# 0xPabloxx/3d-pointcloud-orientation-estimation

Measured on AMD Instinct MI355X. Metric: clouds/sec fwd+bwd, pointnet_pp_vonMises N=1024, higher is better.
Workload: dtype f32; 1 GPU; configs[1]: models/pointnet_pp_vonMises.py single-peak KL, N=1024, batch=32 per GPU, fwd+loss+bwd+allreduce+Adam, random-init weights (seed 42), device-side centre sampling; per_gpu_batch=32, global_batch=32, points=1024, parallelism=single, launch=hipGraph(fwd+loss+bwd) + eager all-reduce/Adam (the update clears the gradients)

## Files before the change

### 3d-pointcloud-orientation-estimation_amd/csrc/gemm_wsd3_kernels.hip

```cpp
#include <stdlib.h>

#include "kernels.h"
#include "split_prims.h"

namespace pnpp {

typedef __attribute__((address_space(3))) volatile unsigned wd3_flag;
__device__ int g_wsd3_timeouts;
__device__ __forceinline__ bool wd3_wait(wd3_flag *f, unsigned target) {
    bool ok = true;
    unsigned spins = 0;
    while ((unsigned)__builtin_amdgcn_readfirstlane((int)*f) < target) {
        __builtin_amdgcn_s_sleep(1);
        if (++spins > (1u << 16)) {
            ok = false;
            break;
        }
    }
    asm volatile("" ::: "memory");
    return ok;
}
__device__ __forceinline__ void wd3_post(wd3_flag *f, unsigned v) {
    asm volatile("s_waitcnt lgkmcnt(0)" ::: "memory");
    *f = v;
}

#ifdef PNPP_STAMPS
__device__ unsigned long long g_wsd3_stamps[2][2][8];
#define WD3_STAMP(i)                                                   \
    if (st_on) {                                                       \
        const unsigned long long st_t = __builtin_amdgcn_s_memtime();  \
        st_acc[i] += st_t - st_last;                                   \
        st_last = st_t;                                                \
    }
#else
#define WD3_STAMP(i)
#endif

template <int KD, int BN, bool HANDOFF>
struct Wsd3Lds {
    static constexpr int WPLANE = BN * KD * 2, APLANE = 32 * 128, ABUF = 3 * APLANE, APAIR = 2 * ABUF, BFR = 2 * 3 * 64 * 16;
    static constexpr int OFF_IMG = 3 * WPLANE, OFF_CST = OFF_IMG + 4 * APAIR, OFF_BFR = OFF_CST + 3 * KD * 4;
    static constexpr int OFF_FLG = OFF_BFR + (HANDOFF ? 4 * BFR : 0), END = OFF_FLG + 64;
};

template <int KD, int BN, int AM>
__global__ void __launch_bounds__(512, 1)
gemm_wsd3_kernel(const AOperand A, const float *__restrict__ W, int ldw, int M, int Nout, int ncol, const Epilogue E) {
    constexpr int NC = KD / 64, CT = KD / 32;
    static_assert(BN == 32, "one column tile per workgroup: the consumer wave holds dW (KD x 32) and the dA tile");
    constexpr bool SPLITDW = true;
    constexpr int CTC = SPLITDW ? CT / 2 : CT;
    constexpr bool HANDOFF = KD == 128;
    constexpr bool DW2 = KD == 128 && AM == A_DZ_POOL;
    constexpr bool ACC2 = true;
    constexpr int WPITCH = KD * 2, WPLANE = BN * WPITCH;
    constexpr int APLANE = 32 * 128, ABUF = 3 * APLANE;
    constexpr int APAIR = 2 * ABUF;
    using LY = Wsd3Lds<KD, BN, HANDOFF>;
    constexpr int BFR = LY::BFR;
    constexpr int OFF_IMG = LY::OFF_IMG, OFF_CST = LY::OFF_CST, OFF_BFR = LY::OFF_BFR, OFF_FLG = LY::OFF_FLG;
    static_assert(NC % 2 == 0, "chunk k of a strip uses buffer k & 1");
    extern __shared__ __attribute__((aligned(16))) unsigned char lds3[];
    unsigned char *Wp = lds3;
    float *Tc = reinterpret_cast<float *>(lds3 + OFF_CST);
    const int tid = threadIdx.x, lane = tid & 63, wave = __builtin_amdgcn_readfirstlane(tid >> 6);
    const bool producer = wave < 4;
    const int pair = wave & 3;
    unsigned char *Ap = lds3 + OFF_IMG + pair * APAIR;
    uint4 *Bf = reinterpret_cast<uint4 *>(lds3 + OFF_BFR + pair * BFR) + lane;
    wd3_flag *f_ready = (wd3_flag *)(lds3 + OFF_FLG) + 2 * pair, *f_done = f_ready + 1;
    const int l31 = lane & 31, lh = lane >> 5;
    auto xw = [](int n) { return n & 15; };

    const int nworkers = gridDim.x / ncol;
    int col_blk = blockIdx.x % ncol, worker = blockIdx.x / ncol;
    if ((nworkers & 7) == 0) {
        const int xcd = blockIdx.x & 7, i = blockIdx.x >> 3;
        col_blk = i % ncol, worker = (i / ncol) * 8 + xcd;
    }
    const int n0 = col_blk * BN;
    const int nstrips = M / 32, stride = nworkers * 4;
    int strip = worker * 4 + pair;
    const __amdgpu_buffer_rsrc_t resNull = sp_buf_rsrc_null(A.z);
    const __amdgpu_buffer_rsrc_t resP = sp_buf_rsrc(E.zp);
    const unsigned oq = 4u * ((unsigned)(4 * lh) * (unsigned)Nout + (unsigned)(n0 + l31));
    auto quni = [&](int r) -> unsigned { return 4u * (unsigned)(((r & 3) + 8 * (r >> 2)) * Nout); };
    const float e_sc = E.scale[n0 + l31], e_sh = E.shift[n0 + l31];
    unsigned tbase[2];
    {
        const int gi = lane & 15, qq = gi >> 2, pp = gi & 3, g1 = (lane >> 4) & 1;
#pragma unroll
        for (int b = 0; b < 2; ++b) {
            const int r = 8 * b + 4 * lh + qq, ch = 2 * g1 + (pp >> 1);
            tbase[b] = (unsigned)(r * 128 + 16 * (ch ^ sp_swz_row(r)) + 8 * (pp & 1));
        }
    }
    auto tofs = [&](int it, int s, int b) -> unsigned { return (tbase[b] ^ (unsigned)(it * 64)) + (unsigned)(s * 2048); };
    auto act_fragments = [&](const float (&z)[16], uint4 (&bfr)[2][3]) {
        float act[16];
#pragma unroll
        for (int r = 0; r < 16; ++r) act[r] = fmaxf(fmaf(z[r], e_sc, e_sh), 0.f);
#pragma unroll
        for (int s = 0; s < 2; ++s) {
            f32x4 v0, v1;
            v0[0] = act[8 * s + 0], v0[1] = act[8 * s + 1], v0[2] = act[8 * s + 2], v0[3] = act[8 * s + 3];
            v1[0] = act[8 * s + 4], v1[1] = act[8 * s + 5], v1[2] = act[8 * s + 6], v1[3] = act[8 * s + 7];
            uint2 h0, m0, l0, h1, m1, l1;
            sp_split4(v0, h0, m0, l0);
            sp_split4(v1, h1, m1, l1);
            bfr[s][0] = make_uint4(h0.x, h0.y, h1.x, h1.y);
            bfr[s][1] = make_uint4(m0.x, m0.y, m1.x, m1.y);
            bfr[s][2] = make_uint4(l0.x, l0.y, l1.x, l1.y);
        }
    };
    auto dw_tile = [&](const unsigned char *Ab, int it, const uint4 (&bfr)[2][3], f32x16 &dwl, f32x16 &dwsm, auto last) {
#pragma unroll
        for (int s = 0; s < 2; ++s) {
            uint4 ta[3];
#pragma unroll
            for (int p = 0; p < 3; ++p) {
                const uint2 lo = sp_tr_b64(Ab + p * APLANE + tofs(it, s, 0)), hi = sp_tr_b64(Ab + p * APLANE + tofs(it, s, 1));
                ta[p] = make_uint4(lo.x, lo.y, hi.x, hi.y);
            }
            if (s == 1) last();
            const bf16x8 ah = sp_op(ta[0]), am = sp_op(ta[1]), al = sp_op(ta[2]);
            const bf16x8 bh = sp_op(bfr[s][0]), bm = sp_op(bfr[s][1]), bl = sp_op(bfr[s][2]);
            f32x16 d = DW2 ? dwsm : dwl;
            d = __builtin_amdgcn_mfma_f32_32x32x16_bf16(al, bh, d, 0, 0, 0);
            d = __builtin_amdgcn_mfma_f32_32x32x16_bf16(ah, bl, d, 0, 0, 0);
            d = __builtin_amdgcn_mfma_f32_32x32x16_bf16(am, bm, d, 0, 0, 0);
            d = __builtin_amdgcn_mfma_f32_32x32x16_bf16(am, bh, d, 0, 0, 0);
            d = __builtin_amdgcn_mfma_f32_32x32x16_bf16(ah, bm, d, 0, 0, 0);
            if constexpr (DW2) {
                dwsm = d;
                dwl = __builtin_amdgcn_mfma_f32_32x32x16_bf16(ah, bh, dwl, 0, 0, 0);
            } else {
                dwl = __builtin_amdgcn_mfma_f32_32x32x16_bf16(ah, bh, d, 0, 0, 0);
            }
        }
    };

    if (tid < 8) ((wd3_flag *)(lds3 + OFF_FLG))[tid] = 0u;
    for (int c = tid; c < KD; c += 512) {
        const float g = A.cst[c], mu = A.cst[A.C + c], is = A.cst[2 * A.C + c], c1 = A.cst[3 * A.C + c], c2 = A.cst[4 * A.C + c];
        const float a = -g * is * c2;
        Tc[c] = g, Tc[KD + c] = a, Tc[2 * KD + c] = -g * c1 - a * mu;
    }
    {
        constexpr int NWF = (KD / 4) * BN / 512;
        f32x4 tw[NWF];
#pragma unroll
        for (int j = 0; j < NWF; ++j) {
            const int f = tid + 512 * j, nl = f % BN, k4 = 4 * (f / BN);
#pragma unroll
            for (int e = 0; e < 4; ++e) tw[j][e] = W[(size_t)(k4 + e) * ldw + n0 + nl];
        }
#pragma unroll
        for (int j = 0; j < NWF; ++j) {
            const int f = tid + 512 * j, nl = f % BN, k4 = 4 * (f / BN);
            uint2 h, m, l;
            sp_split4(tw[j], h, m, l);
            unsigned char *dst = Wp + nl * WPITCH + 16 * ((k4 >> 3) ^ xw(nl)) + 2 * (k4 & 7);
            *reinterpret_cast<uint2 *>(dst) = h;
            *reinterpret_cast<uint2 *>(dst + WPLANE) = m;
            *reinterpret_cast<uint2 *>(dst + 2 * WPLANE) = l;
        }
    }
    __syncthreads();

#ifdef PNPP_STAMPS
    const bool st_on = blockIdx.x == 8 && pair == 0;
    unsigned long long st_acc[8] = {0, 0, 0, 0, 0, 0, 0, 0};
    unsigned long long st_last = __builtin_amdgcn_s_memtime();
#endif
    f32x16 dw[CTC], dws[DW2 ? CTC : 1];
    double s1 = 0.0, s2 = 0.0;
    bool timed_out = false;

    if (producer) {
        const int q = lane & 15, q4 = 4 * q, rb = lane >> 4;
        const __amdgpu_buffer_rsrc_t resZ = sp_buf_rsrc(A.z), resY = sp_buf_rsrc(A.a), resI = sp_buf_rsrc(A.arg);
        const unsigned oa0 = 4u * ((unsigned)rb * (unsigned)KD + (unsigned)q4);
        f32x4 rz[2][8], ry[AM == A_DZ ? 2 : 1][8], rdm[2];
        int4 rarg[2];
        auto fetch_chunk = [&](bool have, int s, int c) {
            const __amdgpu_buffer_rsrc_t rZ = have ? resZ : resNull, rY = have ? resY : resNull, rI = have ? resI : resNull;
            const unsigned so = (unsigned)s * (32u * KD * 4u) + 256u * (unsigned)c;
#pragma unroll
            for (int i = 0; i < 8; ++i) {
                rz[c & 1][i] = sp_buf_load4(rZ, oa0, so + (unsigned)i * (4u * KD * 4u));
                if constexpr (AM == A_DZ) ry[c & 1][i] = sp_buf_load4(rY, oa0, so + (unsigned)i * (4u * KD * 4u));
            }
            if constexpr (AM == A_DZ_POOL) {
                const unsigned sg = (unsigned)s * (KD * 4u) + 256u * (unsigned)c;
                rdm[c & 1] = sp_buf_load4(rY, 4u * (unsigned)q4, sg);
                rarg[c & 1] = __builtin_bit_cast(int4, sp_buf_load4(rI, 4u * (unsigned)q4, sg));
            }
        };
        float zn[16];
        {
            const bool have = strip < nstrips;
            fetch_chunk(have, strip, 0);
            fetch_chunk(have, strip, 1);
            const __amdgpu_buffer_rsrc_t rP = have ? resP : resNull;
#pragma unroll
            for (int r = 0; r < 16; ++r) zn[r] = sp_buf_load1(rP, oq, (unsigned)strip * (32u * (unsigned)Nout * 4u) + quni(r));
        }
        unsigned wofs[4];
#pragma unroll
        for (int i = 0; i < 4; ++i) wofs[i] = (unsigned)(rb * 128 + 16 * ((q >> 1) ^ sp_swz_row(rb + 4 * i)) + 8 * (q & 1));
        if constexpr (SPLITDW) {
#pragma unroll
            for (int i = 0; i < CTC; ++i)
#pragma unroll
                for (int r = 0; r < 16; ++r) dw[i][r] = 0.f;
            if constexpr (DW2) {
#pragma unroll
                for (int i = 0; i < CTC; ++i)
#pragma unroll
                    for (int r = 0; r < 16; ++r) dws[i][r] = 0.f;
            }
        }
        unsigned kbase = 0;
        for (; strip < nstrips; strip += stride, kbase += NC) {
            const bool more = strip + stride < nstrips;
            const int snext = strip + stride;
            uint4 bfr[2][3];
            act_fragments(zn, bfr);
            {
                const __amdgpu_buffer_rsrc_t nP = more ? resP : resNull;
                const unsigned sn_off = (unsigned)snext * (32u * (unsigned)Nout * 4u);
#pragma unroll
                for (int r = 0; r < 16; ++r) zn[r] = sp_buf_load1(nP, oq, sn_off + quni(r));
            }
            if constexpr (HANDOFF) {
                if (kbase >= 2) timed_out = timed_out || !wd3_wait(f_done, kbase - 1);
#pragma unroll
                for (int s = 0; s < 2; ++s)
#pragma unroll
                    for (int p3 = 0; p3 < 3; ++p3) Bf[(s * 3 + p3) * 64] = bfr[s][p3];
            }
#pragma unroll
            for (int c = 0; c < NC; ++c) {
                unsigned char *Ab = Ap + (c & 1) * ABUF;
                const float4 cg = *reinterpret_cast<const float4 *>(Tc + 64 * c + q4), ca = *reinterpret_cast<const float4 *>(Tc + KD + 64 * c + q4);
                const float4 cb = *reinterpret_cast<const float4 *>(Tc + 2 * KD + 64 * c + q4);
                f32x4 dm = {0.f, 0.f, 0.f, 0.f};
                int4 ar = make_int4(-1, -1, -1, -1);
                if constexpr (AM == A_DZ_POOL) dm = rdm[c & 1], ar = rarg[c & 1];
                float4 bt;
                bt.x = fmaf(cg.x, dm[0], cb.x), bt.y = fmaf(cg.y, dm[1], cb.y), bt.z = fmaf(cg.z, dm[2], cb.z), bt.w = fmaf(cg.w, dm[3], cb.w);
                auto dz4 = [&](int i) -> f32x4 {
                    const f32x4 z = rz[c & 1][i];
                    const int r = rb + 4 * i;
                    f32x4 v;
                    if constexpr (AM == A_DZ) {
                        const f32x4 dy = ry[c & 1][i];
                        v[0] = fmaf(cg.x, dy[0], fmaf(ca.x, z[0], cb.x)), v[1] = fmaf(cg.y, dy[1], fmaf(ca.y, z[1], cb.y));
                        v[2] = fmaf(cg.z, dy[2], fmaf(ca.z, z[2], cb.z)), v[3] = fmaf(cg.w, dy[3], fmaf(ca.w, z[3], cb.w));
                    } else {
                        v[0] = fmaf(ca.x, z[0], r == ar.x ? bt.x : cb.x), v[1] = fmaf(ca.y, z[1], r == ar.y ? bt.y : cb.y);
                        v[2] = fmaf(ca.z, z[2], r == ar.z ? bt.z : cb.z), v[3] = fmaf(ca.w, z[3], r == ar.w ? bt.w : cb.w);
                    }
                    return v;
                };
                if constexpr (AM == A_DZ_POOL && !SPLITDW) {
                    uint2 ph[8], pm[8], pl[8];
#pragma unroll
                    for (int i = 0; i < 8; ++i) sp_split4(dz4(i), ph[i], pm[i], pl[i]);
                    WD3_STAMP(0)
                    if (c + 2 < NC) fetch_chunk(true, strip, c + 2);
                    else fetch_chunk(more, snext, c + 2 - NC);
                    if (kbase + c >= 2) timed_out = timed_out || !wd3_wait(f_done, kbase + c - 1);
                    WD3_STAMP(1)
#pragma unroll
                    for (int i = 0; i < 8; ++i) {
                        unsigned char *dst = Ab + wofs[i & 3] + i * 512;
                        *reinterpret_cast<uint2 *>(dst) = ph[i];
                        *reinterpret_cast<uint2 *>(dst + APLANE) = pm[i];
                        *reinterpret_cast<uint2 *>(dst + 2 * APLANE) = pl[i];
                    }
                } else {
                    if (kbase + c >= 2) timed_out = timed_out || !wd3_wait(f_done, kbase + c - 1);
                    WD3_STAMP(1)
#pragma unroll
                    for (int i = 0; i < 8; ++i) {
                        uint2 h, m, l;
                        sp_split4(dz4(i), h, m, l);
                        unsigned char *dst = Ab + wofs[i & 3] + i * 512;
                        *reinterpret_cast<uint2 *>(dst) = h;
                        *reinterpret_cast<uint2 *>(dst + APLANE) = m;
                        *reinterpret_cast<uint2 *>(dst + 2 * APLANE) = l;
                    }
                    WD3_STAMP(0)
                    if (c + 2 < NC) fetch_chunk(true, strip, c + 2);
                    else fetch_chunk(more, snext, c + 2 - NC);
                }
                wd3_post(f_ready, kbase + c + 1);
                WD3_STAMP(2)
                if constexpr (SPLITDW) {
                    if (c >= NC / 2) {
#pragma unroll
                        for (int it = 0; it < 2; ++it) dw_tile(Ab, it, bfr, dw[2 * c + it - CTC], dws[DW2 ? 2 * c + it - CTC : 0], [] {});
                    }
                }
            }
        }
    } else {
#pragma unroll
        for (int i = 0; i < CTC; ++i)
#pragma unroll
            for (int r = 0; r < 16; ++r) dw[i][r] = 0.f;
        if constexpr (DW2) {
#pragma unroll
            for (int i = 0; i < CTC; ++i)
#pragma unroll
                for (int r = 0; r < 16; ++r) dws[i][r] = 0.f;
        }
        const __amdgpu_buffer_rsrc_t resC = sp_buf_rsrc(E.c);
        const float e_mu = E.mu[n0 + l31], e_is = E.istd[n0 + l31];
        float zq[16];
        const unsigned arow = (unsigned)(l31 * 128);
        const int ax = sp_swz_row(l31);
        const unsigned char *brow = Wp + l31 * WPITCH;
        const int bx = xw(l31);
        float zn[16];
        if constexpr (!HANDOFF) {
            const __amdgpu_buffer_rsrc_t rP = strip < nstrips ? resP : resNull;
#pragma unroll
            for (int r = 0; r < 16; ++r) zn[r] = sp_buf_load1(rP, oq, (unsigned)strip * (32u * (unsigned)Nout * 4u) + quni(r));
        }
        unsigned kbase = 0;
        for (; strip < nstrips; strip += stride, kbase += NC) {
            const bool more = strip + stride < nstrips;
            uint4 bfr[2][3];
            if constexpr (HANDOFF) {
                const unsigned sq_off = (unsigned)strip * (32u * (unsigned)Nout * 4u);
#pragma unroll
                for (int r = 0; r < 16; ++r) zq[r] = sp_buf_load1(resP, oq, sq_off + quni(r));
            } else {
#pragma unroll
                for (int r = 0; r < 16; ++r) zq[r] = zn[r];
                const __amdgpu_buffer_rsrc_t nP = more ? resP : resNull;
                const unsigned sn_off = (unsigned)(strip + stride) * (32u * (unsigned)Nout * 4u);
#pragma unroll
                for (int r = 0; r < 16; ++r) zn[r] = sp_buf_load1(nP, oq, sn_off + quni(r));
                act_fragments(zq, bfr);
            }
            f32x16 acc, accs;
#pragma unroll
            for (int r = 0; r < 16; ++r) acc[r] = 0.f;
            if constexpr (ACC2) {
#pragma unroll
                for (int r = 0; r < 16; ++r) accs[r] = 0.f;
            }
            WD3_STAMP(3)
#pragma unroll
            for (int c = 0; c < NC; ++c) {
                const unsigned char *Ab = Ap + (c & 1) * ABUF;
                timed_out = timed_out || !wd3_wait(f_ready, kbase + c + 1);
                if constexpr (HANDOFF) {
                    if (c == 0) {
#pragma unroll
                        for (int s = 0; s < 2; ++s)
#pragma unroll
                            for (int p3 = 0; p3 < 3; ++p3) bfr[s][p3] = Bf[(s * 3 + p3) * 64];
                    }
                }
                WD3_STAMP(4)
#pragma unroll
                for (int t = 0; t < 4; ++t) {
                    const int g = 2 * t + lh;
                    uint4 fa[3], fb[3];
#pragma unroll
                    for (int p = 0; p < 3; ++p) {
                        fa[p] = *reinterpret_cast<const uint4 *>(Ab + p * APLANE + arow + 16 * (g ^ ax));
                        fb[p] = *reinterpret_cast<const uint4 *>(brow + p * WPLANE + 16 * ((8 * c + g) ^ bx));
                    }
                    const bf16x8 ah = sp_op(fa[0]), am = sp_op(fa[1]), al = sp_op(fa[2]);
                    const bf16x8 bh = sp_op(fb[0]), bm = sp_op(fb[1]), bl = sp_op(fb[2]);
                    f32x16 d = ACC2 ? accs : acc;
                    d = __builtin_amdgcn_mfma_f32_32x32x16_bf16(al, bh, d, 0, 0, 0);
                    d = __builtin_amdgcn_mfma_f32_32x32x16_bf16(ah, bl, d, 0, 0, 0);
                    d = __builtin_amdgcn_mfma_f32_32x32x16_bf16(am, bm, d, 0, 0, 0);
                    d = __builtin_amdgcn_mfma_f32_32x32x16_bf16(am, bh, d, 0, 0, 0);
                    d = __builtin_amdgcn_mfma_f32_32x32x16_bf16(ah, bm, d, 0, 0, 0);
                    if constexpr (ACC2) {
                        accs = d;
                        acc = __builtin_amdgcn_mfma_f32_32x32x16_bf16(ah, bh, acc, 0, 0, 0);
                    } else {
                        acc = __builtin_amdgcn_mfma_f32_32x32x16_bf16(ah, bh, d, 0, 0, 0);
                    }
                }
                WD3_STAMP(5)
                if (!SPLITDW || c < NC / 2) {
                    dw_tile(Ab, 0, bfr, dw[2 * c < CTC ? 2 * c : 0], dws[DW2 ? (2 * c < CTC ? 2 * c : 0) : 0], [] {});
                    dw_tile(Ab, 1, bfr, dw[2 * c + 1 < CTC ? 2 * c + 1 : 0], dws[DW2 ? (2 * c + 1 < CTC ? 2 * c + 1 : 0) : 0],
                            [&] { wd3_post(f_done, kbase + c + 1); });
                } else {
                    wd3_post(f_done, kbase + c + 1);
                }
                WD3_STAMP(6)
            }
            {
                const unsigned sc_off = (unsigned)strip * (32u * (unsigned)Nout * 4u);
                float t1 = 0.f, t2 = 0.f;
#pragma unroll
                for (int r = 0; r < 16; ++r) {
                    const float v = fmaf(zq[r], e_sc, e_sh) > 0.f ? (ACC2 ? acc[r] + accs[r] : acc[r]) : 0.f;
                    __builtin_amdgcn_raw_buffer_store_b32(__builtin_bit_cast(unsigned, v), resC, (int)oq, (int)(sc_off + quni(r)), 0);
                    t1 += v;
                    t2 = fmaf(v, zq[r], t2);
                }
                const double d1 = (double)t1;
                s1 += d1, s2 += (double)e_is * ((double)t2 - (double)e_mu * d1);
            }
            WD3_STAMP(7)
        }
    }
#ifdef PNPP_STAMPS
    if (st_on && lane == 0)
#pragma unroll
        for (int i = 0; i < 8; ++i) g_wsd3_stamps[KD == 256][producer ? 0 : 1][i] += st_acc[i];
#endif
    if (timed_out && lane == 0) atomicExch(&g_wsd3_timeouts, 1);

    __syncthreads();
    f32x4 *red = reinterpret_cast<f32x4 *>(lds3);
    double *dred = reinterpret_cast<double *>(lds3 + CT * 4 * 4 * 64 * 16);
    if (!producer || SPLITDW) {
        const int t0 = producer ? CTC : 0;
#pragma unroll
        for (int i = 0; i < CTC; ++i)
#pragma unroll
            for (int r4 = 0; r4 < 4; ++r4) {
                f32x4 v;
#pragma unroll
                for (int e = 0; e < 4; ++e) v[e] = DW2 ? dw[i][4 * r4 + e] + dws[DW2 ? i : 0][4 * r4 + e] : dw[i][4 * r4 + e];
                red[(((t0 + i) * 4 + pair) * 4 + r4) * 64 + lane] = v;
            }
    }
    if (!producer) {
        const double a = s1 + shfl_xor_f64(s1, 32), b = s2 + shfl_xor_f64(s2, 32);
        if (lh == 0) dred[(pair * 2 + 0) * BN + l31] = a, dred[(pair * 2 + 1) * BN + l31] = b;
    }
    __syncthreads();
    {
        float *wb = E.dwslab + (size_t)worker * KD * E.dw_ld + n0;
        for (int t = wave; t < CT; t += 8) {
#pragma unroll
            for (int r4 = 0; r4 < 4; ++r4) {
                const f32x4 a0 = red[((t * 4 + 0) * 4 + r4) * 64 + lane], a1 = red[((t * 4 + 1) * 4 + r4) * 64 + lane];
                const f32x4 a2 = red[((t * 4 + 2) * 4 + r4) * 64 + lane], a3 = red[((t * 4 + 3) * 4 + r4) * 64 + lane];
                const int c0 = t * 32 + 8 * r4 + 4 * lh;
                float *o = wb + (size_t)c0 * E.dw_ld + l31;
#pragma unroll
                for (int e = 0; e < 4; ++e) o[(size_t)e * E.dw_ld] = (a0[e] + a1[e]) + (a2[e] + a3[e]);
            }
        }
        if (tid < 2 * BN) {
            const int which = tid / BN, cl = tid % BN;
            const double t = (dred[(0 * 2 + which) * BN + cl] + dred[(1 * 2 + which) * BN + cl]) +
                             (dred[(2 * 2 + which) * BN + cl] + dred[(3 * 2 + which) * BN + cl]);
            E.slab[((size_t)worker * 2 + which) * Nout + n0 + cl] = t;
        }
    }
}

template <int KD, int BN, int AM>
static void wsd3_launch(const AOperand &A, const BOperand &B, int M, int Nout, const Epilogue &E, int workers, int ncol, hipStream_t st) {
    constexpr size_t main_b = Wsd3Lds<KD, BN, KD != 256>::END;
    constexpr size_t red_b = (size_t)(KD / 32) * (BN / 32) * 4 * 4 * 64 * 16 + (size_t)4 * 2 * BN * 8;
    constexpr size_t lds = main_b > red_b ? main_b : red_b;
    static_assert(lds <= 160 * 1024, "LDS budget");
    auto kfn = gemm_wsd3_kernel<KD, BN, AM>;
    static bool granted = false;
    if (!granted) {
        (void)hipFuncSetAttribute((const void *)kfn, hipFuncAttributeMaxDynamicSharedMemorySize, (int)lds);
        granted = true;
    }
    hipLaunchKernelGGL(kfn, dim3(workers * ncol), dim3(512), lds, st, A, B.b, B.ldb, M, Nout, ncol, E);
}

bool wsd3_applies(const AOperand &A, const BOperand &B, int M, int Nout, int Kd, const Epilogue &E) {
    if (!split_products() || matmul_precision() != 0) return false;
    const bool pooled = A.mode == A_DZ_POOL && A.K == 32 && ((Kd == 128 && Nout == 64) || (Kd == 256 && Nout == 128));
    const bool dense = A.mode == A_DZ && Kd == 128 && Nout == 128 && A.a;
    if (M < 8192 || M % 32 != 0 || !(pooled || dense)) return false;
    if (E.mode != E_MASK_STATS || !E.dwslab || E.dw_ld < Nout) return false;
    if (B.trans || B.perm_D >= 0 || (B.rows > 0 && B.rows != Kd) || B.ldb < Nout) return false;
    if (A.lda != Kd || A.C != Kd || E.ldc != Nout) return false;
    if ((((uintptr_t)A.a | (uintptr_t)A.z | (uintptr_t)E.zp | (uintptr_t)E.c | (uintptr_t)A.cst) & 15) != 0) return false;
    if (A.mode == A_DZ_POOL && (((uintptr_t)A.arg) & 15) != 0) return false;
    if ((unsigned long long)M * (unsigned)Kd * 4ull >= 0xfffffff0ull) return false;
    return true;
}

bool try_launch_wsd3(const AOperand &A, const BOperand &B, int M, int Nout, int Kd, const Epilogue &E, int *nslab, hipStream_t st, int *rc,
                     int *dw_slabs) {
    *rc = PNPP_OK;
    if (!dw_slabs || !wsd3_applies(A, B, M, Nout, Kd, E)) return false;
    const int nstrips = M / 32, ncol = Nout / 32;
    int workers = 256 / ncol;
    if (workers * 4 > nstrips) workers = (nstrips + 3) / 4;
    if (workers > kMaxStatBlocks) workers = kMaxStatBlocks;
    if (nslab) *nslab = workers;
    *dw_slabs = workers;
    ProfScope ps(st, "gemm_wsd3_kernel<%d,32,A%d> M=%d N=%d K=%d grid=%dx1", Kd, A.mode, M, Nout, Kd, workers * ncol);
    if (Kd == 256) wsd3_launch<256, 32, A_DZ_POOL>(A, B, M, Nout, E, workers, ncol, st);
    else if (A.mode == A_DZ_POOL) wsd3_launch<128, 32, A_DZ_POOL>(A, B, M, Nout, E, workers, ncol, st);
    else wsd3_launch<128, 32, A_DZ>(A, B, M, Nout, E, workers, ncol, st);
    if (hipGetLastError() != hipSuccess) {
        set_error("gemm_wsd3: launch failed");
        *rc = PNPP_ERR_LAUNCH;
    }
    return true;
}

#ifdef PNPP_STAMPS
#define WD3_STAMPS_BIT 64u
#else
#define WD3_STAMPS_BIT 0u
#endif
#ifdef WD3_PRIO
#define WD3_PRIO_BIT 256u
#else
#define WD3_PRIO_BIT 0u
#endif
unsigned wsd3_build_flags() { return WD3_STAMPS_BIT | WD3_PRIO_BIT; }

int wsd3_timeouts() {
    int v = 0;
    (void)hipMemcpyFromSymbol(&v, HIP_SYMBOL(g_wsd3_timeouts), sizeof(int));
    return v;
}

}

extern "C" int pnpp_debug_wsd3_timeouts(void) { return pnpp::wsd3_timeouts(); }
#ifdef PNPP_STAMPS
extern "C" int pnpp_debug_wsd3_stamps(unsigned long long *out32, int reset) {
    if (reset) {
        unsigned long long z[32] = {0};
        hipMemcpyToSymbol(HIP_SYMBOL(pnpp::g_wsd3_stamps), z, sizeof(z));
    } else {
        hipDeviceSynchronize();
        hipMemcpyFromSymbol(out32, HIP_SYMBOL(pnpp::g_wsd3_stamps), 32 * sizeof(unsigned long long));
    }
    return 0;
}
#endif
```

Before: 58850 clouds/s.

## Share each A strip across two column tiles per workgroup in wsd3 backward GEMM

Each workgroup now covers two 32-wide output column tiles instead of one. The two wave pairs in a column-pair group share one A image: each producer splits alternate K-chunks of the same strip, and consumers of both column tiles read it. This cuts redundant global loads and split/convert work on the dZ activations per column, halves the number of strips in flight per workgroup, and doubles the slabs per block. In exchange it adds cross-pair flag synchronisation (ready/done/fragment flags), a reworked dW reduction layout, and a changed grid/slab count.

```diff
diff --git a/3d-pointcloud-orientation-estimation_amd/csrc/gemm_wsd3_kernels.hip b/3d-pointcloud-orientation-estimation_amd/csrc/gemm_wsd3_kernels.hip
--- a/3d-pointcloud-orientation-estimation_amd/csrc/gemm_wsd3_kernels.hip
+++ b/3d-pointcloud-orientation-estimation_amd/csrc/gemm_wsd3_kernels.hip
@@ -1,4 +1,6 @@
 #include <stdlib.h>
+
+#include <type_traits>
 
 #include "kernels.h"
 #include "split_prims.h"
@@ -39,49 +41,56 @@
 
 template <int KD, int BN, bool HANDOFF>
 struct Wsd3Lds {
-    static constexpr int WPLANE = BN * KD * 2, APLANE = 32 * 128, ABUF = 3 * APLANE, APAIR = 2 * ABUF, BFR = 2 * 3 * 64 * 16;
-    static constexpr int OFF_IMG = 3 * WPLANE, OFF_CST = OFF_IMG + 4 * APAIR, OFF_BFR = OFF_CST + 3 * KD * 4;
-    static constexpr int OFF_FLG = OFF_BFR + (HANDOFF ? 4 * BFR : 0), END = OFF_FLG + 64;
+    static constexpr int CB = 2;
+    static constexpr int WPLANE = CB * BN * KD * 2, APLANE = 32 * 128, ABUF = 3 * APLANE, ACPL = 2 * ABUF, BFR = 2 * 3 * 64 * 16;
+    static constexpr int OFF_IMG = 3 * WPLANE, OFF_CST = OFF_IMG + 2 * ACPL, OFF_BFR = OFF_CST + 3 * KD * 4;
+    static constexpr int NFLG = 3 * 4;
+    static constexpr int OFF_FLG = OFF_BFR + (HANDOFF ? 4 * BFR : 0), END = OFF_FLG + (NFLG * 4 + 63) / 64 * 64;
+    static constexpr int RED = (KD / 32) * CB * 2 * 4 * 64 * 16, TAIL = RED + 4 * 2 * BN * 8;
+    static constexpr int BYTES = END > TAIL ? END : TAIL;
 };
 
 template <int KD, int BN, int AM>
 __global__ void __launch_bounds__(512, 1)
-gemm_wsd3_kernel(const AOperand A, const float *__restrict__ W, int ldw, int M, int Nout, int ncol, const Epilogue E) {
+gemm_wsd3_kernel(const AOperand A, const float *__restrict__ W, int ldw, int M, int Nout, int ncg, const Epilogue E) {
     constexpr int NC = KD / 64, CT = KD / 32;
-    static_assert(BN == 32, "one column tile per workgroup: the consumer wave holds dW (KD x 32) and the dA tile");
-    constexpr bool SPLITDW = true;
-    constexpr int CTC = SPLITDW ? CT / 2 : CT;
+    static_assert(BN == 32, "one column tile per wave pair: the consumer wave holds half of dW (KD x 32) and the dA tile");
+    constexpr int NCP = NC / 2;
+    constexpr int AHEAD = 2 / NCP;
+    constexpr int CTC = CT / 2;
     constexpr bool HANDOFF = KD == 128;
     constexpr bool DW2 = KD == 128 && AM == A_DZ_POOL;
     constexpr bool ACC2 = true;
-    constexpr int WPITCH = KD * 2, WPLANE = BN * WPITCH;
-    constexpr int APLANE = 32 * 128, ABUF = 3 * APLANE;
-    constexpr int APAIR = 2 * ABUF;
     using LY = Wsd3Lds<KD, BN, HANDOFF>;
+    constexpr int CB = LY::CB;
+    constexpr int WPITCH = KD * 2, WPLANE = LY::WPLANE;
+    constexpr int APLANE = LY::APLANE, ABUF = LY::ABUF;
     constexpr int BFR = LY::BFR;
     constexpr int OFF_IMG = LY::OFF_IMG, OFF_CST = LY::OFF_CST, OFF_BFR = LY::OFF_BFR, OFF_FLG = LY::OFF_FLG;
-    static_assert(NC % 2 == 0, "chunk k of a strip uses buffer k & 1");
+    static_assert(NC % 2 == 0 && (NCP == 1 || NCP == 2), "chunk k of a strip uses buffer k & 1 and belongs to producer k & 1");
     extern __shared__ __attribute__((aligned(16))) unsigned char lds3[];
     unsigned char *Wp = lds3;
     float *Tc = reinterpret_cast<float *>(lds3 + OFF_CST);
     const int tid = threadIdx.x, lane = tid & 63, wave = __builtin_amdgcn_readfirstlane(tid >> 6);
     const bool producer = wave < 4;
-    const int pair = wave & 3;
-    unsigned char *Ap = lds3 + OFF_IMG + pair * APAIR;
+    const int pair = wave & 3, cpl = pair >> 1, sub = pair & 1;
+    unsigned char *Ap = lds3 + OFF_IMG + cpl * LY::ACPL;
     uint4 *Bf = reinterpret_cast<uint4 *>(lds3 + OFF_BFR + pair * BFR) + lane;
-    wd3_flag *f_ready = (wd3_flag *)(lds3 + OFF_FLG) + 2 * pair, *f_done = f_ready + 1;
+    wd3_flag *flg = (wd3_flag *)(lds3 + OFF_FLG);
+    wd3_flag *f_rdy = flg + 2 * cpl, *f_don = flg + 4 + 2 * cpl, *f_frg = flg + 8 + pair;
     const int l31 = lane & 31, lh = lane >> 5;
     auto xw = [](int n) { return n & 15; };
 
-    const int nworkers = gridDim.x / ncol;
-    int col_blk = blockIdx.x % ncol, worker = blockIdx.x / ncol;
+    const int nworkers = gridDim.x / ncg;
+    int col_grp = blockIdx.x % ncg, worker = blockIdx.x / ncg;
     if ((nworkers & 7) == 0) {
         const int xcd = blockIdx.x & 7, i = blockIdx.x >> 3;
-        col_blk = i % ncol, worker = (i / ncol) * 8 + xcd;
-    }
-    const int n0 = col_blk * BN;
-    const int nstrips = M / 32, stride = nworkers * 4;
-    int strip = worker * 4 + pair;
+        col_grp = i % ncg, worker = (i / ncg) * 8 + xcd;
+    }
+    const int nw0 = col_grp * CB * BN;
+    const int n0 = nw0 + sub * BN;
+    const int nstrips = M / 32, stride = nworkers * 2;
+    int strip = worker * 2 + cpl;
     const __amdgpu_buffer_rsrc_t resNull = sp_buf_rsrc_null(A.z);
     const __amdgpu_buffer_rsrc_t resP = sp_buf_rsrc(E.zp);
     const unsigned oq = 4u * ((unsigned)(4 * lh) * (unsigned)Nout + (unsigned)(n0 + l31));
@@ -141,24 +150,24 @@
         }
     };
 
-    if (tid < 8) ((wd3_flag *)(lds3 + OFF_FLG))[tid] = 0u;
+    if (tid < LY::NFLG) flg[tid] = 0u;
     for (int c = tid; c < KD; c += 512) {
         const float g = A.cst[c], mu = A.cst[A.C + c], is = A.cst[2 * A.C + c], c1 = A.cst[3 * A.C + c], c2 = A.cst[4 * A.C + c];
         const float a = -g * is * c2;
         Tc[c] = g, Tc[KD + c] = a, Tc[2 * KD + c] = -g * c1 - a * mu;
     }
     {
-        constexpr int NWF = (KD / 4) * BN / 512;
+        constexpr int PN = CB * BN, NWF = (KD / 4) * PN / 512;
         f32x4 tw[NWF];
 #pragma unroll
         for (int j = 0; j < NWF; ++j) {
-            const int f = tid + 512 * j, nl = f % BN, k4 = 4 * (f / BN);
-#pragma unroll
-            for (int e = 0; e < 4; ++e) tw[j][e] = W[(size_t)(k4 + e) * ldw + n0 + nl];
+            const int f = tid + 512 * j, nl = f % PN, k4 = 4 * (f / PN);
+#pragma unroll
+            for (int e = 0; e < 4; ++e) tw[j][e] = W[(size_t)(k4 + e) * ldw + nw0 + nl];
         }
 #pragma unroll
         for (int j = 0; j < NWF; ++j) {
-            const int f = tid + 512 * j, nl = f % BN, k4 = 4 * (f / BN);
+            const int f = tid + 512 * j, nl = f % PN, k4 = 4 * (f / PN);
             uint2 h, m, l;
             sp_split4(tw[j], h, m, l);
             unsigned char *dst = Wp + nl * WPITCH + 16 * ((k4 >> 3) ^ xw(nl)) + 2 * (k4 & 7);
@@ -175,6 +184,16 @@
     unsigned long long st_last = __builtin_amdgcn_s_memtime();
 #endif
     f32x16 dw[CTC], dws[DW2 ? CTC : 1];
+#pragma unroll
+    for (int i = 0; i < CTC; ++i)
+#pragma unroll
+        for (int r = 0; r < 16; ++r) dw[i][r] = 0.f;
+    if constexpr (DW2) {
+#pragma unroll
+        for (int i = 0; i < CTC; ++i)
+#pragma unroll
+            for (int r = 0; r < 16; ++r) dws[i][r] = 0.f;
+    }
     double s1 = 0.0, s2 = 0.0;
     bool timed_out = false;
 
@@ -184,48 +203,39 @@
         const unsigned oa0 = 4u * ((unsigned)rb * (unsigned)KD + (unsigned)q4);
         f32x4 rz[2][8], ry[AM == A_DZ ? 2 : 1][8], rdm[2];
         int4 rarg[2];
-        auto fetch_chunk = [&](bool have, int s, int c) {
+        auto fetch_chunk = [&](int s, int c, int set) {
+            const bool have = s < nstrips;
             const __amdgpu_buffer_rsrc_t rZ = have ? resZ : resNull, rY = have ? resY : resNull, rI = have ? resI : resNull;
             const unsigned so = (unsigned)s * (32u * KD * 4u) + 256u * (unsigned)c;
 #pragma unroll
             for (int i = 0; i < 8; ++i) {
-                rz[c & 1][i] = sp_buf_load4(rZ, oa0, so + (unsigned)i * (4u * KD * 4u));
-                if constexpr (AM == A_DZ) ry[c & 1][i] = sp_buf_load4(rY, oa0, so + (unsigned)i * (4u * KD * 4u));
+                rz[set][i] = sp_buf_load4(rZ, oa0, so + (unsigned)i * (4u * KD * 4u));
+                if constexpr (AM == A_DZ) ry[set][i] = sp_buf_load4(rY, oa0, so + (unsigned)i * (4u * KD * 4u));
             }
             if constexpr (AM == A_DZ_POOL) {
                 const unsigned sg = (unsigned)s * (KD * 4u) + 256u * (unsigned)c;
-                rdm[c & 1] = sp_buf_load4(rY, 4u * (unsigned)q4, sg);
-                rarg[c & 1] = __builtin_bit_cast(int4, sp_buf_load4(rI, 4u * (unsigned)q4, sg));
+                rdm[set] = sp_buf_load4(rY, 4u * (unsigned)q4, sg);
+                rarg[set] = __builtin_bit_cast(int4, sp_buf_load4(rI, 4u * (unsigned)q4, sg));
             }
         };
         float zn[16];
         {
-            const bool have = strip < nstrips;
-            fetch_chunk(have, strip, 0);
-            fetch_chunk(have, strip, 1);
-            const __amdgpu_buffer_rsrc_t rP = have ? resP : resNull;
+            fetch_chunk(strip, sub, 0);
+            if constexpr (NCP == 2) fetch_chunk(strip, 2 + sub, 1);
+            else fetch_chunk(strip + stride, sub, 1);
+            const __amdgpu_buffer_rsrc_t rP = strip < nstrips ? resP : resNull;
 #pragma unroll
             for (int r = 0; r < 16; ++r) zn[r] = sp_buf_load1(rP, oq, (unsigned)strip * (32u * (unsigned)Nout * 4u) + quni(r));
         }
         unsigned wofs[4];
 #pragma unroll
         for (int i = 0; i < 4; ++i) wofs[i] = (unsigned)(rb * 128 + 16 * ((q >> 1) ^ sp_swz_row(rb + 4 * i)) + 8 * (q & 1));
-        if constexpr (SPLITDW) {
-#pragma unroll
-            for (int i = 0; i < CTC; ++i)
-#pragma unroll
-                for (int r = 0; r < 16; ++r) dw[i][r] = 0.f;
-            if constexpr (DW2) {
-#pragma unroll
-                for (int i = 0; i < CTC; ++i)
-#pragma unroll
-                    for (int r = 0; r < 16; ++r) dws[i][r] = 0.f;
-            }
-        }
+        unsigned char *Ab = Ap + sub * ABUF;
         unsigned kbase = 0;
-        for (; strip < nstrips; strip += stride, kbase += NC) {
-            const bool more = strip + stride < nstrips;
+        unsigned pub = 0;
+        auto p_strip = [&](auto PAR) {
             const int snext = strip + stride;
+            const bool more = snext < nstrips;
             uint4 bfr[2][3];
             act_fragments(zn, bfr);
             {
@@ -235,28 +245,30 @@
                 for (int r = 0; r < 16; ++r) zn[r] = sp_buf_load1(nP, oq, sn_off + quni(r));
             }
             if constexpr (HANDOFF) {
-                if (kbase >= 2) timed_out = timed_out || !wd3_wait(f_done, kbase - 1);
+                if (kbase >= NC) timed_out = timed_out || !wd3_wait(f_don + sub, kbase - NC + 1);
 #pragma unroll
                 for (int s = 0; s < 2; ++s)
 #pragma unroll
                     for (int p3 = 0; p3 < 3; ++p3) Bf[(s * 3 + p3) * 64] = bfr[s][p3];
-            }
-#pragma unroll
-            for (int c = 0; c < NC; ++c) {
-                unsigned char *Ab = Ap + (c & 1) * ABUF;
+                wd3_post(f_frg, kbase / NC + 1);
+            }
+#pragma unroll
+            for (int j = 0; j < NCP; ++j) {
+                const int set = NCP == 2 ? j : decltype(PAR)::value;
+                const int c = 2 * j + sub;
                 const float4 cg = *reinterpret_cast<const float4 *>(Tc + 64 * c + q4), ca = *reinterpret_cast<const float4 *>(Tc + KD + 64 * c + q4);
                 const float4 cb = *reinterpret_cast<const float4 *>(Tc + 2 * KD + 64 * c + q4);
                 f32x4 dm = {0.f, 0.f, 0.f, 0.f};
                 int4 ar = make_int4(-1, -1, -1, -1);
-                if constexpr (AM == A_DZ_POOL) dm = rdm[c & 1], ar = rarg[c & 1];
+                if constexpr (AM == A_DZ_POOL) dm = rdm[set], ar = rarg[set];
                 float4 bt;
                 bt.x = fmaf(cg.x, dm[0], cb.x), bt.y = fmaf(cg.y, dm[1], cb.y), bt.z = fmaf(cg.z, dm[2], cb.z), bt.w = fmaf(cg.w, dm[3], cb.w);
                 auto dz4 = [&](int i) -> f32x4 {
-                    const f32x4 z = rz[c & 1][i];
+                    const f32x4 z = rz[set][i];
                     const int r = rb + 4 * i;
                     f32x4 v;
                     if constexpr (AM == A_DZ) {
-                        const f32x4 dy = ry[c & 1][i];
+                        const f32x4 dy = ry[set][i];
                         v[0] = fmaf(cg.x, dy[0], fmaf(ca.x, z[0], cb.x)), v[1] = fmaf(cg.y, dy[1], fmaf(ca.y, z[1], cb.y));
                         v[2] = fmaf(cg.z, dy[2], fmaf(ca.z, z[2], cb.z)), v[3] = fmaf(cg.w, dy[3], fmaf(ca.w, z[3], cb.w));
                     } else {
@@ -265,65 +277,44 @@
                     }
                     return v;
                 };
-                if constexpr (AM == A_DZ_POOL && !SPLITDW) {
-                    uint2 ph[8], pm[8], pl[8];
-#pragma unroll
-                    for (int i = 0; i < 8; ++i) sp_split4(dz4(i), ph[i], pm[i], pl[i]);
-                    WD3_STAMP(0)
-                    if (c + 2 < NC) fetch_chunk(true, strip, c + 2);
-                    else fetch_chunk(more, snext, c + 2 - NC);
-                    if (kbase + c >= 2) timed_out = timed_out || !wd3_wait(f_done, kbase + c - 1);
-                    WD3_STAMP(1)
-#pragma unroll
-                    for (int i = 0; i < 8; ++i) {
-                        unsigned char *dst = Ab + wofs[i & 3] + i * 512;
-                        *reinterpret_cast<uint2 *>(dst) = ph[i];
-                        *reinterpret_cast<uint2 *>(dst + APLANE) = pm[i];
-                        *reinterpret_cast<uint2 *>(dst + 2 * APLANE) = pl[i];
-                    }
-                } else {
-                    if (kbase + c >= 2) timed_out = timed_out || !wd3_wait(f_done, kbase + c - 1);
-                    WD3_STAMP(1)
-#pragma unroll
-                    for (int i = 0; i < 8; ++i) {
-                        uint2 h, m, l;
-                        sp_split4(dz4(i), h, m, l);
-                        unsigned char *dst = Ab + wofs[i & 3] + i * 512;
-                        *reinterpret_cast<uint2 *>(dst) = h;
-                        *reinterpret_cast<uint2 *>(dst + APLANE) = m;
-                        *reinterpret_cast<uint2 *>(dst + 2 * APLANE) = l;
-                    }
-                    WD3_STAMP(0)
-                    if (c + 2 < NC) fetch_chunk(true, strip, c + 2);
-                    else fetch_chunk(more, snext, c + 2 - NC);
+                if (kbase + c >= 2) {
+                    timed_out = timed_out || !wd3_wait(f_don + 0, kbase + c - 1);
+                    timed_out = timed_out || !wd3_wait(f_don + 1, kbase + c - 1);
                 }
-                wd3_post(f_ready, kbase + c + 1);
+                WD3_STAMP(1)
+#pragma unroll
+                for (int i = 0; i < 8; ++i) {
+                    uint2 h, m, l;
+                    sp_split4(dz4(i), h, m, l);
+                    unsigned char *dst = Ab + wofs[i & 3] + i * 512;
+                    *reinterpret_cast<uint2 *>(dst) = h;
+                    *reinterpret_cast<uint2 *>(dst + APLANE) = m;
+                    *reinterpret_cast<uint2 *>(dst + 2 * APLANE) = l;
+                }
+                WD3_STAMP(0)
+                fetch_chunk(strip + AHEAD * stride, c, set);
+                wd3_post(f_rdy + sub, ++pub);
                 WD3_STAMP(2)
-                if constexpr (SPLITDW) {
-                    if (c >= NC / 2) {
-#pragma unroll
-                        for (int it = 0; it < 2; ++it) dw_tile(Ab, it, bfr, dw[2 * c + it - CTC], dws[DW2 ? 2 * c + it - CTC : 0], [] {});
-                    }
-                }
+#pragma unroll
+                for (int it = 0; it < 2; ++it) dw_tile(Ab, it, bfr, dw[2 * j + it], dws[DW2 ? 2 * j + it : 0], [] {});
+            }
+        };
+        while (strip < nstrips) {
+            p_strip(std::integral_constant<int, 0>{});
+            strip += stride, kbase += NC;
+            if constexpr (NCP == 1) {
+                if (strip >= nstrips) break;
+                p_strip(std::integral_constant<int, 1>{});
+                strip += stride, kbase += NC;
             }
         }
     } else {
-#pragma unroll
-        for (int i = 0; i < CTC; ++i)
-#pragma unroll
-            for (int r = 0; r < 16; ++r) dw[i][r] = 0.f;
-        if constexpr (DW2) {
-#pragma unroll
-            for (int i = 0; i < CTC; ++i)
-#pragma unroll
-                for (int r = 0; r < 16; ++r) dws[i][r] = 0.f;
-        }
         const __amdgpu_buffer_rsrc_t resC = sp_buf_rsrc(E.c);
         const float e_mu = E.mu[n0 + l31], e_is = E.istd[n0 + l31];
         float zq[16];
         const unsigned arow = (unsigned)(l31 * 128);
         const int ax = sp_swz_row(l31);
-        const unsigned char *brow = Wp + l31 * WPITCH;
+        const unsigned char *brow = Wp + (sub * BN + l31) * WPITCH;
         const int bx = xw(l31);
         float zn[16];
         if constexpr (!HANDOFF) {
@@ -331,8 +322,8 @@
 #pragma unroll
             for (int r = 0; r < 16; ++r) zn[r] = sp_buf_load1(rP, oq, (unsigned)strip * (32u * (unsigned)Nout * 4u) + quni(r));
         }
-        unsigned kbase = 0;
-        for (; strip < nstrips; strip += stride, kbase += NC) {
+        unsigned kbase = 0, sidx = 0;
+        for (; strip < nstrips; strip += stride, kbase += NC, ++sidx) {
             const bool more = strip + stride < nstrips;
             uint4 bfr[2][3];
             if constexpr (HANDOFF) {
@@ -359,9 +350,10 @@
 #pragma unroll
             for (int c = 0; c < NC; ++c) {
                 const unsigned char *Ab = Ap + (c & 1) * ABUF;
-                timed_out = timed_out || !wd3_wait(f_ready, kbase + c + 1);
+                timed_out = timed_out || !wd3_wait(f_rdy + (c & 1), sidx * NCP + (c >> 1) + 1);
                 if constexpr (HANDOFF) {
                     if (c == 0) {
+                        timed_out = timed_out || !wd3_wait(f_frg, sidx + 1);
 #pragma unroll
                         for (int s = 0; s < 2; ++s)
 #pragma unroll
@@ -394,12 +386,12 @@
                     }
                 }
                 WD3_STAMP(5)
-                if (!SPLITDW || c < NC / 2) {
-                    dw_tile(Ab, 0, bfr, dw[2 * c < CTC ? 2 * c : 0], dws[DW2 ? (2 * c < CTC ? 2 * c : 0) : 0], [] {});
-                    dw_tile(Ab, 1, bfr, dw[2 * c + 1 < CTC ? 2 * c + 1 : 0], dws[DW2 ? (2 * c + 1 < CTC ? 2 * c + 1 : 0) : 0],
-                            [&] { wd3_post(f_done, kbase + c + 1); });
+                if ((c & 1) != sub) {
+                    const int i0 = 2 * (c >> 1);
+                    dw_tile(Ab, 0, bfr, dw[i0], dws[DW2 ? i0 : 0], [] {});
+                    dw_tile(Ab, 1, bfr, dw[i0 + 1], dws[DW2 ? i0 + 1 : 0], [&] { wd3_post(f_don + sub, kbase + c + 1); });
                 } else {
-                    wd3_post(f_done, kbase + c + 1);
+                    wd3_post(f_don + sub, kbase + c + 1);
                 }
                 WD3_STAMP(6)
             }
@@ -428,18 +420,20 @@
 
     __syncthreads();
     f32x4 *red = reinterpret_cast<f32x4 *>(lds3);
-    double *dred = reinterpret_cast<double *>(lds3 + CT * 4 * 4 * 64 * 16);
-    if (!producer || SPLITDW) {
-        const int t0 = producer ? CTC : 0;
-#pragma unroll
-        for (int i = 0; i < CTC; ++i)
+    double *dred = reinterpret_cast<double *>(lds3 + LY::RED);
+    {
+        const int par = producer ? sub : 1 - sub;
+#pragma unroll
+        for (int i = 0; i < CTC; ++i) {
+            const int t = 2 * (2 * (i >> 1) + par) + (i & 1);
 #pragma unroll
             for (int r4 = 0; r4 < 4; ++r4) {
                 f32x4 v;
 #pragma unroll
                 for (int e = 0; e < 4; ++e) v[e] = DW2 ? dw[i][4 * r4 + e] + dws[DW2 ? i : 0][4 * r4 + e] : dw[i][4 * r4 + e];
-                red[(((t0 + i) * 4 + pair) * 4 + r4) * 64 + lane] = v;
-            }
+                red[(((t * CB + sub) * 2 + cpl) * 4 + r4) * 64 + lane] = v;
+            }
+        }
     }
     if (!producer) {
         const double a = s1 + shfl_xor_f64(s1, 32), b = s2 + shfl_xor_f64(s2, 32);
@@ -447,32 +441,29 @@
     }
     __syncthreads();
     {
-        float *wb = E.dwslab + (size_t)worker * KD * E.dw_ld + n0;
-        for (int t = wave; t < CT; t += 8) {
+        float *wb = E.dwslab + (size_t)worker * KD * E.dw_ld + nw0;
+        for (int u = wave; u < CT * CB; u += 8) {
+            const int t = u / CB, b = u % CB;
 #pragma unroll
             for (int r4 = 0; r4 < 4; ++r4) {
-                const f32x4 a0 = red[((t * 4 + 0) * 4 + r4) * 64 + lane], a1 = red[((t * 4 + 1) * 4 + r4) * 64 + lane];
-                const f32x4 a2 = red[((t * 4 + 2) * 4 + r4) * 64 + lane], a3 = red[((t * 4 + 3) * 4 + r4) * 64 + lane];
+                const f32x4 a0 = red[((u * 2 + 0) * 4 + r4) * 64 + lane], a1 = red[((u * 2 + 1) * 4 + r4) * 64 + lane];
                 const int c0 = t * 32 + 8 * r4 + 4 * lh;
-                float *o = wb + (size_t)c0 * E.dw_ld + l31;
-#pragma unroll
-                for (int e = 0; e < 4; ++e) o[(size_t)e * E.dw_ld] = (a0[e] + a1[e]) + (a2[e] + a3[e]);
-            }
-        }
-        if (tid < 2 * BN) {
-            const int which = tid / BN, cl = tid % BN;
-            const double t = (dred[(0 * 2 + which) * BN + cl] + dred[(1 * 2 + which) * BN + cl]) +
-                             (dred[(2 * 2 + which) * BN + cl] + dred[(3 * 2 + which) * BN + cl]);
-            E.slab[((size_t)worker * 2 + which) * Nout + n0 + cl] = t;
+                float *o = wb + (size_t)c0 * E.dw_ld + b * BN + l31;
+#pragma unroll
+                for (int e = 0; e < 4; ++e) o[(size_t)e * E.dw_ld] = a0[e] + a1[e];
+            }
+        }
+        if (tid < 2 * CB * BN) {
+            const int which = tid / (CB * BN), cl = tid % (CB * BN), b = cl / BN, c31 = cl % BN;
+            const double t = dred[((0 + b) * 2 + which) * BN + c31] + dred[((2 + b) * 2 + which) * BN + c31];
+            E.slab[((size_t)worker * 2 + which) * Nout + nw0 + cl] = t;
         }
     }
 }
 
 template <int KD, int BN, int AM>
-static void wsd3_launch(const AOperand &A, const BOperand &B, int M, int Nout, const Epilogue &E, int workers, int ncol, hipStream_t st) {
-    constexpr size_t main_b = Wsd3Lds<KD, BN, KD != 256>::END;
-    constexpr size_t red_b = (size_t)(KD / 32) * (BN / 32) * 4 * 4 * 64 * 16 + (size_t)4 * 2 * BN * 8;
-    constexpr size_t lds = main_b > red_b ? main_b : red_b;
+static void wsd3_launch(const AOperand &A, const BOperand &B, int M, int Nout, const Epilogue &E, int grid, int ncg, hipStream_t st) {
+    constexpr size_t lds = Wsd3Lds<KD, BN, KD != 256>::BYTES;
     static_assert(lds <= 160 * 1024, "LDS budget");
     auto kfn = gemm_wsd3_kernel<KD, BN, AM>;
     static bool granted = false;
@@ -480,7 +471,7 @@
         (void)hipFuncSetAttribute((const void *)kfn, hipFuncAttributeMaxDynamicSharedMemorySize, (int)lds);
         granted = true;
     }
-    hipLaunchKernelGGL(kfn, dim3(workers * ncol), dim3(512), lds, st, A, B.b, B.ldb, M, Nout, ncol, E);
+    hipLaunchKernelGGL(kfn, dim3(grid), dim3(512), lds, st, A, B.b, B.ldb, M, Nout, ncg, E);
 }
 
 bool wsd3_applies(const AOperand &A, const BOperand &B, int M, int Nout, int Kd, const Epilogue &E) {
@@ -501,16 +492,17 @@
                      int *dw_slabs) {
     *rc = PNPP_OK;
     if (!dw_slabs || !wsd3_applies(A, B, M, Nout, Kd, E)) return false;
-    const int nstrips = M / 32, ncol = Nout / 32;
+    const int nstrips = M / 32, ncol = Nout / 32, ncg = ncol / 2;
     int workers = 256 / ncol;
     if (workers * 4 > nstrips) workers = (nstrips + 3) / 4;
-    if (workers > kMaxStatBlocks) workers = kMaxStatBlocks;
-    if (nslab) *nslab = workers;
-    *dw_slabs = workers;
-    ProfScope ps(st, "gemm_wsd3_kernel<%d,32,A%d> M=%d N=%d K=%d grid=%dx1", Kd, A.mode, M, Nout, Kd, workers * ncol);
-    if (Kd == 256) wsd3_launch<256, 32, A_DZ_POOL>(A, B, M, Nout, E, workers, ncol, st);
-    else if (A.mode == A_DZ_POOL) wsd3_launch<128, 32, A_DZ_POOL>(A, B, M, Nout, E, workers, ncol, st);
-    else wsd3_launch<128, 32, A_DZ>(A, B, M, Nout, E, workers, ncol, st);
+    if (2 * workers > kMaxStatBlocks) workers = kMaxStatBlocks / 2;
+    const int grid = workers * ncol, rows = grid / ncg;
+    if (nslab) *nslab = rows;
+    *dw_slabs = rows;
+    ProfScope ps(st, "gemm_wsd3_kernel<%d,32,A%d> M=%d N=%d K=%d grid=%dx1", Kd, A.mode, M, Nout, Kd, grid);
+    if (Kd == 256) wsd3_launch<256, 32, A_DZ_POOL>(A, B, M, Nout, E, grid, ncg, st);
+    else if (A.mode == A_DZ_POOL) wsd3_launch<128, 32, A_DZ_POOL>(A, B, M, Nout, E, grid, ncg, st);
+    else wsd3_launch<128, 32, A_DZ>(A, B, M, Nout, E, grid, ncg, st);
     if (hipGetLastError() != hipSuccess) {
         set_error("gemm_wsd3: launch failed");
         *rc = PNPP_ERR_LAUNCH;
```

Result: no change. 58390 clouds/s (-0.8%).
